# rsokolovskii/fl_scaling_sc_ldpc

Hardware: AMD Instinct MI355X
Metric: MC codeword trials/sec, (4,8) SC-LDPC L=50 N=1000 eps=0.48 full BP (higher is better)
Workload: dtype u32

## Files before the change

fl_scaling_sc_ldpc_amd/csrc/sampler_v2.hip:

```cpp
#include "common.h"
#include "kernel_util.h"
#include "philox.h"
#include <algorithm>
#include <cstdlib>

namespace {

using scldpc_dev::philox4x32_10;
using scldpc_dev::wave_inclusive_scan;

constexpr int kThreads = 1024;
constexpr int kWaves = kThreads / 64;
constexpr int kMaxDoped = 32;
constexpr int kWorkCap = 1024;

struct S2Args {
    int L, cns_pos, vns_pos, n, S, D, nb, shift, sbits, nw;
    int ntrials;
    int force_exact;
    int ndoped;
    int doped[kMaxDoped];
    uint32_t seed_lo, seed_hi;
    unsigned long long trial0;
    uint32_t thresh;
    int off_gpk, off_fix, off_stage, off_wsum;
    uint16_t *vn_adj16;
    uint16_t *cn_adj16;
    uint32_t *chan;
};

template <int KMAX, int ROWS, int CNMODE, bool PERSIST = false>
__global__ __launch_bounds__(kThreads, KMAX == 1 ? 8 : 4) __attribute__((amdgpu_num_sgpr(72))) void sample_philox_v2_kernel(const S2Args a)
{
    constexpr int DV = 4, DC_SHIFT = 3, E = 4 * KMAX;
    extern __shared__ uint32_t lds[];
    uint32_t *hist = lds;
    uint32_t *gpk = lds + a.off_gpk;
    uint16_t *fix = reinterpret_cast<uint16_t *>(lds + a.off_fix);
    uint16_t *stage = reinterpret_cast<uint16_t *>(lds + a.off_stage);
    uint32_t *wsum = lds + a.off_wsum;
    uint32_t *wl = wsum + 32;

    const int tid = threadIdx.x, lane = tid & 63, wave = tid >> 6;
    const int S = a.S, nb = a.nb;
    const int ncalls = S >> 2;
    const int kshift = a.shift - 2;
    const uint32_t lowmask = (1u << kshift) - 1u;
    bool own[KMAX];
#pragma unroll
    for (int k = 0; k < KMAX; k++) own[k] = tid + k * kThreads < ncalls;
    auto sock = [&](int e) { return (uint32_t)((tid + (e >> 2) * kThreads) * 4 + (e & 3)); };
    auto stage_entry = [&](int p, uint32_t sck) -> uint16_t {
        const int u = (int)(sck & 3u), t = (int)(sck >> 2);
        if ((unsigned)(p - u) >= (unsigned)a.L) return (uint16_t)0xFFFFu;
        return CNMODE == 1 ? (uint16_t)((p - u) * a.vns_pos + t) : (uint16_t)sck;
    };

    auto nib_sum = [](uint32_t x) {
        const uint32_t v = (x & 0x0F0Fu) + ((x >> 4) & 0x0F0Fu);
        return (v + (v >> 8)) & 0xFFu;
    };
    auto load_words = [&](uint32_t (&x)[ROWS]) {
        if constexpr (ROWS % 4 == 0) {
#pragma unroll
            for (int r = 0; r < ROWS / 4; r++) {
                const uint4 q = reinterpret_cast<const uint4 *>(hist)[tid * (ROWS / 4) + r];
                x[4 * r] = q.x; x[4 * r + 1] = q.y; x[4 * r + 2] = q.z; x[4 * r + 3] = q.w;
            }
        } else if constexpr (ROWS == 2) { const uint2 q = reinterpret_cast<const uint2 *>(hist)[tid]; x[0] = q.x; x[1] = q.y; }
        else x[0] = hist[tid];
    };
    auto store_words = [&](const uint32_t (&x)[ROWS]) {
        if constexpr (ROWS % 4 == 0) {
#pragma unroll
            for (int r = 0; r < ROWS / 4; r++)
                reinterpret_cast<uint4 *>(hist)[tid * (ROWS / 4) + r] = make_uint4(x[4 * r], x[4 * r + 1], x[4 * r + 2], x[4 * r + 3]);
        } else if constexpr (ROWS == 2) reinterpret_cast<uint2 *>(hist)[tid] = make_uint2(x[0], x[1]);
        else hist[tid] = x[0];
    };
    STAMP_DECL
    for (int b = tid; b < nb; b += kThreads) hist[b] = 0;
    if (tid == 0) { wsum[kWaves] = 0; wsum[kWaves + 1] = 0; }
    __syncthreads();
    auto sample_trial = [&](const int tr) {
    const unsigned long long trial = a.trial0 + (unsigned long long)tr;
    const uint32_t t_lo = (uint32_t)trial, t_hi = (uint32_t)(trial >> 32);
    uint32_t rowP[KMAX], rowQ[KMAX], rowR[KMAX];
#pragma unroll
    for (int k = 0; k < KMAX; k++) rowP[k] = rowQ[k] = rowR[k] = 0;
    uint32_t nxt[E];
#pragma unroll
    for (int k = 0; k < KMAX; k++) {
        uint32_t r[4] = {0, 0, 0, 0};
        if (own[k]) philox4x32_10((uint32_t)(tid + k * kThreads), 0u, t_lo, t_hi, a.seed_lo, a.seed_hi, r);
#pragma unroll
        for (int u = 0; u < 4; u++) nxt[4 * k + u] = r[u];
    }
    for (int p = 0; p < a.D; p++) {
        STAMP(0);
        uint32_t key[E], slot[E], crowded = 0;
#pragma unroll
        for (int e = 0; e < E; e++) {
            key[e] = nxt[e];
            const uint32_t b = key[e] >> kshift, sh = (b & 3u) * 4u;
            slot[e] = (atomicAdd(&hist[b >> 2], (own[e >> 2] ? 1u : 0u) << sh) >> sh) & 0xFu;
            crowded = max(crowded, slot[e]);
        }
        if (crowded >= 15u) wsum[kWaves + 1] = 1u;
        __syncthreads();
        STAMP(1);

        {
            uint32_t x[ROWS], v[ROWS], tot = 0;
            load_words(x);
#pragma unroll
            for (int r = 0; r < ROWS; r++) v[r] = 0;
            if constexpr (ROWS % 2 == 0) {
#pragma unroll
                for (int r = 0; r < ROWS; r += 2) {
                    const uint32_t y = x[r] | (x[r + 1] << 16);
                    const uint32_t sb = (y & 0x0F0F0F0Fu) + ((y >> 4) & 0x0F0F0F0Fu);
                    v[r] = (sb & 0xFFu) + ((sb >> 8) & 0xFFu);
                    v[r + 1] = ((sb >> 16) & 0xFFu) + (sb >> 24);
                    tot += v[r] + v[r + 1];
                }
            } else {
                static_assert(ROWS == 1 || ROWS % 2 == 0, "ROWS is 1, 2, 4 or 8");
                v[0] = nib_sum(x[0]);
                tot = v[0];
            }
            const uint32_t inc = wave_inclusive_scan(tot);
            if (lane == 63) wsum[wave] = inc;
            __syncthreads();
            const uint32_t wt = lane < kWaves ? wsum[lane] : 0u;
            const uint32_t winc = wave_inclusive_scan(wt);
            uint32_t pre = inc - tot + (uint32_t)__builtin_amdgcn_readlane((int)(winc - wt), wave);
#pragma unroll
            for (int r = 0; r < ROWS; r++) { x[r] |= pre << 16; pre += v[r]; }
            store_words(x);
        }
        __syncthreads();
        STAMP(2);

        if (wsum[kWaves + 1] == 0u) {
            uint32_t h[E], rk[E], g0a[E], cnta[E], smask = 0;
#pragma unroll
            for (int e = 0; e < E; e++) h[e] = hist[own[e >> 2] ? (key[e] >> kshift) >> 2 : 0u];
#pragma unroll
            for (int e = 0; e < E; e++) {
                const uint32_t k4 = ((key[e] >> kshift) & 3u) * 4u, x = h[e];
                const uint32_t below = x & ((1u << k4) - 1u);
                g0a[e] = (x >> 16) + (below & 0xFu) + ((below >> 4) & 0xFu) + ((below >> 8) & 0xFu);
                cnta[e] = (x >> k4) & 0xFu;
                rk[e] = g0a[e] + slot[e];
                if (own[e >> 2] && ((g0a[e] + cnta[e] - 1u) >> DC_SHIFT) != (g0a[e] >> DC_SHIFT)) smask |= 1u << e;
            }
            while (smask) {
                const uint32_t e = (uint32_t)__ffs((int)smask) - 1u;
                smask &= smask - 1u;
                uint32_t ky = key[0], sl = slot[0], g0 = g0a[0], cnt = cnta[0];
#pragma unroll
                for (int f = 1; f < E; f++)
                    if (e == (uint32_t)f) { ky = key[f]; sl = slot[f]; g0 = g0a[f]; cnt = cnta[f]; }
                const uint32_t pk = ((ky & lowmask) << a.sbits) | (uint32_t)((tid + (int)(e >> 2) * kThreads) * 4 + (int)(e & 3u));
                gpk[g0 + sl] = pk;
                const int w = atomicAdd(reinterpret_cast<int *>(&wsum[kWaves]), 1);
                if (w < kWorkCap) { wl[2 * w] = g0 | (cnt << 16) | (sl << 20); wl[2 * w + 1] = pk; }
            }
#pragma unroll
            for (int k = 0; k < KMAX; k++) {
                if (!own[k]) continue;
                uint2 v;
                v.x = (rk[4 * k] >> DC_SHIFT) | ((rk[4 * k + 1] >> DC_SHIFT) << 16);
                v.y = (rk[4 * k + 2] >> DC_SHIFT) | ((rk[4 * k + 3] >> DC_SHIFT) << 16);
                reinterpret_cast<uint2 *>(fix)[tid + k * kThreads] = v;
            }
            if constexpr (CNMODE != 0) {
#pragma unroll
                for (int k = 0; k < KMAX; k++) {
                    if (!own[k]) continue;
#pragma unroll
                    for (int u = 0; u < 4; u++) stage[rk[4 * k + u]] = stage_entry(p, sock(4 * k + u));
                }
            }
        }
        __syncthreads();
        STAMP(3);

        {
            uint32_t z[ROWS];
#pragma unroll
            for (int r = 0; r < ROWS; r++) z[r] = 0;
            store_words(z);
            int nwork = (int)wsum[kWaves];
            const bool exact = wsum[kWaves + 1] != 0u || nwork > kWorkCap || a.force_exact == p || a.force_exact == -2;
            if (exact) {
                nwork = 0;
#pragma unroll
                for (int e = 0; e < E; e++) if (own[e >> 2]) gpk[sock(e)] = key[e];
                __syncthreads();
                uint32_t xr[E];
#pragma unroll
                for (int e = 0; e < E; e++) xr[e] = 0;
                for (int s2 = 0; s2 < S; s2++) {
                    const uint32_t k2 = gpk[s2];
#pragma unroll
                    for (int e = 0; e < E; e++) xr[e] += (k2 < key[e]) || (k2 == key[e] && (uint32_t)s2 < sock(e));
                }
#pragma unroll
                for (int k = 0; k < KMAX; k++) {
                    if (!own[k]) continue;
                    uint2 v;
                    v.x = (xr[4 * k] >> DC_SHIFT) | ((xr[4 * k + 1] >> DC_SHIFT) << 16);
                    v.y = (xr[4 * k + 2] >> DC_SHIFT) | ((xr[4 * k + 3] >> DC_SHIFT) << 16);
                    reinterpret_cast<uint2 *>(fix)[tid + k * kThreads] = v;
                    if constexpr (CNMODE != 0) {
#pragma unroll
                        for (int u = 0; u < 4; u++) stage[xr[4 * k + u]] = stage_entry(p, sock(4 * k + u));
                    }
                }
            }
            for (int w = tid; w < nwork; w += kThreads) {
                const uint32_t ea = wl[2 * w], pk = wl[2 * w + 1];
                const uint32_t g0 = ea & 0xFFFFu, cnt = (ea >> 16) & 0xFu, sl = ea >> 20;
                uint32_t r = g0;
                for (uint32_t m = 0; m < cnt; m++)
                    if (m != sl) r += gpk[g0 + m] < pk;
                const uint32_t sck = pk & ((1u << a.sbits) - 1u);
                if constexpr (CNMODE != 0) stage[r] = stage_entry(p, sck);
                fix[sck] = (uint16_t)(r >> DC_SHIFT);
            }
        }
        if (p + 1 < a.D) {
            uint32_t k_lo = a.seed_lo, k_hi = a.seed_hi;
            asm volatile("" : "+s"(k_lo), "+s"(k_hi));
#pragma unroll
            for (int k = 0; k < KMAX; k++) {
                uint32_t r[4] = {0, 0, 0, 0};
                if (own[k]) philox4x32_10((uint32_t)(tid + k * kThreads), (uint32_t)(p + 1), t_lo, t_hi, k_lo, k_hi, r);
#pragma unroll
                for (int u = 0; u < 4; u++) nxt[4 * k + u] = r[u];
            }
        }
        __syncthreads();
        if (tid == 0) { wsum[kWaves] = 0; wsum[kWaves + 1] = 0; }
        STAMP(4);

        const int qpos = p - (DV - 1);
#pragma unroll
        for (int k = 0; k < KMAX; k++) {
            uint2 c = make_uint2(0u, 0u);
            if (own[k]) c = reinterpret_cast<const uint2 *>(fix)[tid + k * kThreads];
            if (qpos >= 0 && own[k]) {
                const size_t j = (size_t)tr * a.n + (size_t)qpos * a.vns_pos + (size_t)(tid + k * kThreads);
                uint2 v;
                v.x = rowP[k];
                v.y = (rowR[k] >> 16) | (c.y & 0xFFFF0000u);
                reinterpret_cast<uint2 *>(a.vn_adj16)[j] = v;
            }
            rowP[k] = rowQ[k];
            rowQ[k] = (rowR[k] & 0xFFFFu) | (c.x & 0xFFFF0000u);
            rowR[k] = (c.x & 0xFFFFu) | (c.y << 16);
        }
        if constexpr (CNMODE != 0) {
            uint2 *dst = reinterpret_cast<uint2 *>(a.cn_adj16) + ((size_t)tr * a.D + p) * (size_t)(S >> 2);
            const uint2 *src = reinterpret_cast<const uint2 *>(stage);
            for (int w = tid; w < (S >> 2); w += kThreads) dst[w] = src[w];
        }
        STAMP(5);
    }

    uint32_t *chan = a.chan + (size_t)tr * a.nw;
    for (int w = tid; w < a.nw; w += kThreads) {
        uint32_t word = 0;
#pragma unroll
        for (int c = 0; c < 8; c++) {
            uint32_t r[4];
            philox4x32_10((uint32_t)(w * 8 + c), 0x80000000u, t_lo, t_hi, a.seed_lo, a.seed_hi, r);
#pragma unroll
            for (int u = 0; u < 4; u++) word |= (uint32_t)((r[u] >> 1) < a.thresh) << (c * 4 + u);
        }
        const int j0 = w * 32;
        if (j0 + 32 > a.n) word &= (1u << (a.n - j0)) - 1u;
        for (int d = 0; d < a.ndoped; d++) {
            const int lo = max(a.doped[d] * a.vns_pos, j0) - j0, hi = min((a.doped[d] + 1) * a.vns_pos, j0 + 32) - j0;
            if (lo < hi) word &= ~(((hi - lo) == 32 ? 0xFFFFFFFFu : ((1u << (hi - lo)) - 1u)) << lo);
        }
        chan[w] = word;
    }
    STAMP(6);
    };
    if constexpr (PERSIST) {
        for (int tr = blockIdx.x; tr < a.ntrials; tr += gridDim.x) {
            sample_trial(tr);
            __syncthreads();
        }
    } else {
        sample_trial((int)blockIdx.x);
    }
    STAMP_FLUSH();
}


__device__ __forceinline__ uint32_t wl_entry_vn(const S2Args &a, int p, uint32_t sck)
{
    return (uint32_t)((p - (int)(sck & 3u)) * a.vns_pos + (int)(sck >> 2));
}

template <int LG, int CNMODE>
__global__ __launch_bounds__(kThreads, 8) __attribute__((amdgpu_num_sgpr(72))) void sample_philox_v3_kernel(const S2Args a)
{
    constexpr int DV = 4, DC_SHIFT = 3, E = 4;
    constexpr int NB = 1 << LG, ROWS = NB / kThreads;
    constexpr int KSHIFT = 32 - LG - 2;
    constexpr uint32_t LOWMASK = (1u << KSHIFT) - 1u;
    constexpr int SBITS = LG;
    static_assert(ROWS == 1 || ROWS == 2 || ROWS == 4, "one Philox call per thread: at most 4096 sockets per position");
    extern __shared__ uint32_t lds[];
    uint32_t *hist0 = lds;
    uint32_t *gpk = lds + a.off_gpk;
    uint16_t *fix = reinterpret_cast<uint16_t *>(lds + a.off_fix);
    uint16_t *stage = reinterpret_cast<uint16_t *>(lds + a.off_stage);
    uint32_t *wsum = lds + a.off_wsum;
    uint32_t *wl = wsum + 32;

    const int tid = threadIdx.x, lane = tid & 63, wave = tid >> 6;
    const int S = a.S;
    const bool own = tid < (S >> 2);
    const unsigned long long trial = a.trial0 + blockIdx.x;
    const uint32_t t_lo = (uint32_t)trial, t_hi = (uint32_t)(trial >> 32);
    const int tr = blockIdx.x;

    STAMP_DECL
    for (int b = tid; b < 2 * NB; b += kThreads) hist0[b] = 0;
    if (tid < 32) wsum[tid] = 0;
    __syncthreads();

    uint32_t rowP = 0, rowQ = 0, rowR = 0;
    uint32_t key[E] = {0, 0, 0, 0}, slot[E] = {0, 0, 0, 0};
    uint32_t ent0 = CNMODE == 1 ? (uint32_t)tid : (uint32_t)(4 * tid);
    uint32_t vV = (uint32_t)a.vns_pos;
    asm volatile("" : "+v"(vV));

    for (int p = 0; p <= a.D; p++) {
        uint32_t *hc = hist0 + (p & 1) * NB, *hp = hist0 + ((p & 1) ^ 1) * NB;
        const bool live = p < a.D;
        STAMP(0);
        if (p > 0) {
            int nwork = (int)wsum[16];
            const bool exact = wsum[18 + ((p - 1) & 1)] != 0u || nwork > kWorkCap || a.force_exact == p - 1 || a.force_exact == -2;
            if (exact) {
                uint32_t k2[4] = {0, 0, 0, 0};
                uint32_t f_lo = a.seed_lo, f_hi = a.seed_hi;
                asm volatile("" : "+s"(f_lo), "+s"(f_hi));
                if (own) philox4x32_10((uint32_t)tid, (uint32_t)(p - 1), t_lo, t_hi, f_lo, f_hi, k2);
                if (own) { gpk[4 * tid] = k2[0]; gpk[4 * tid + 1] = k2[1]; gpk[4 * tid + 2] = k2[2]; gpk[4 * tid + 3] = k2[3]; }
                __syncthreads();
                uint32_t xr[4] = {0, 0, 0, 0};
                for (int s2 = 0; s2 < S; s2++) {
                    const uint32_t kk = gpk[s2];
#pragma unroll
                    for (int u = 0; u < 4; u++) xr[u] += (kk < k2[u]) || (kk == k2[u] && s2 < 4 * tid + u);
                }
                if (own) {
                    uint2 v;
                    v.x = (xr[0] >> DC_SHIFT) | ((xr[1] >> DC_SHIFT) << 16);
                    v.y = (xr[2] >> DC_SHIFT) | ((xr[3] >> DC_SHIFT) << 16);
                    reinterpret_cast<uint2 *>(fix)[tid] = v;
                    if constexpr (CNMODE != 0) {
#pragma unroll
                        for (int u = 0; u < 4; u++) {
                            const int pu = p - 1 - u;
                            stage[xr[u]] = (unsigned)pu < (unsigned)a.L ? (uint16_t)(CNMODE == 1 ? pu * a.vns_pos + tid : 4 * tid + u) : (uint16_t)0xFFFFu;
                        }
                    }
                }
                nwork = 0;
            }
            for (int w = tid; w < nwork; w += kThreads) {
                const uint32_t ea = wl[2 * w], pk = wl[2 * w + 1];
                const uint32_t g0 = ea & 0xFFFFu, cnt = (ea >> 16) & 0xFu, sl = (ea >> 20) & 0xFu;
                uint32_t r = g0;
                for (uint32_t m = 0; m < cnt; m++)
                    if (m != sl) r += gpk[g0 + m] < pk;
                const uint32_t sck = pk & ((1u << SBITS) - 1u);
                if constexpr (CNMODE != 0) stage[r] = (uint16_t)(ea >> 24 ? 0xFFFFu : (CNMODE == 1 ? wl_entry_vn(a, p - 1, sck) : sck));
                fix[sck] = (uint16_t)(r >> DC_SHIFT);
            }
            {
                if constexpr (ROWS == 4) reinterpret_cast<uint4 *>(hp)[tid] = make_uint4(0u, 0u, 0u, 0u);
                else if constexpr (ROWS == 2) reinterpret_cast<uint2 *>(hp)[tid] = make_uint2(0u, 0u);
                else hp[tid] = 0u;
            }
        }
        STAMP(1);
        if (live) {
            {
                uint32_t k_lo = a.seed_lo, k_hi = a.seed_hi;
                asm volatile("" : "+s"(k_lo), "+s"(k_hi));
                uint32_t r[4] = {0, 0, 0, 0};
                if (own) philox4x32_10((uint32_t)tid, (uint32_t)p, t_lo, t_hi, k_lo, k_hi, r);
#pragma unroll
                for (int u = 0; u < 4; u++) key[u] = r[u];
            }
            uint32_t crowded = 0;
#pragma unroll
            for (int e = 0; e < E; e++) {
                const uint32_t boff = (key[e] >> KSHIFT) & ~3u, sh = (key[e] >> (KSHIFT - 2)) & 12u;
                const uint32_t old = atomicAdd(reinterpret_cast<uint32_t *>(reinterpret_cast<char *>(hc) + boff), (own ? 16u : 0u) << sh);
                slot[e] = (old >> (sh + 4u)) & 0xFu;
                crowded |= slot[e] + 1u;
            }
            if (crowded & 16u) wsum[18 + (p & 1)] = 1u;
        }
        STAMP(2);
        __syncthreads();
        STAMP(3);
        if (tid == 0) { wsum[16] = 0; wsum[18 + ((p & 1) ^ 1)] = 0; }
        if (live) {
            uint32_t x[ROWS], tot = 0, over = 0;
            if constexpr (ROWS == 4) { const uint4 q = reinterpret_cast<const uint4 *>(hc)[tid]; x[0] = q.x; x[1] = q.y; x[2] = q.z; x[3] = q.w; }
            else if constexpr (ROWS == 2) { const uint2 q = reinterpret_cast<const uint2 *>(hc)[tid]; x[0] = q.x; x[1] = q.y; }
            else x[0] = hc[tid];
            uint32_t v[ROWS];
#pragma unroll
            for (int r = 0; r < ROWS; r++) {
                const uint32_t y = x[r] * 0x1111u;
                const uint32_t sb = (x[r] & 0x0F0F0u) + ((x[r] >> 4) & 0x0F0F0u);
                v[r] = ((sb + (sb >> 8)) >> 4) & 0xFFu;
                over |= v[r];
                x[r] = y & 0xFFFF0u;
                tot += v[r];
            }
            if (over & ~15u) wsum[18 + (p & 1)] = 1u;
            const uint32_t inc = wave_inclusive_scan(tot);
            uint32_t pre = inc - tot;
#pragma unroll
            for (int r = 0; r < ROWS; r++) { x[r] |= pre << 20; pre += v[r]; }
            if constexpr (ROWS == 4) reinterpret_cast<uint4 *>(hc)[tid] = make_uint4(x[0], x[1], x[2], x[3]);
            else if constexpr (ROWS == 2) reinterpret_cast<uint2 *>(hc)[tid] = make_uint2(x[0], x[1]);
            else hc[tid] = x[0];
            if (lane == 63) wsum[wave] = inc;
        }
        if (p > 0) {
            const int pp = p - 1, qpos = pp - (DV - 1);
            uint2 c = make_uint2(0u, 0u);
            if (own) c = reinterpret_cast<const uint2 *>(fix)[tid];
            if (qpos >= 0 && own) {
                const size_t j = (size_t)tr * a.n + (size_t)qpos * a.vns_pos + (size_t)tid;
                uint2 vv;
                vv.x = rowP;
                vv.y = (rowR >> 16) | (c.y & 0xFFFF0000u);
                reinterpret_cast<uint2 *>(a.vn_adj16)[j] = vv;
            }
            rowP = rowQ;
            rowQ = (rowR & 0xFFFFu) | (c.x & 0xFFFF0000u);
            rowR = (c.x & 0xFFFFu) | (c.y << 16);
            if constexpr (CNMODE != 0) {
                uint2 *dst = reinterpret_cast<uint2 *>(a.cn_adj16) + ((size_t)tr * a.D + pp) * (size_t)(S >> 2);
                const uint2 *src = reinterpret_cast<const uint2 *>(stage);
                if (own) dst[tid] = src[tid];
            }
        }
        STAMP(4);
        __syncthreads();
        STAMP(5);
        if (live && wsum[18 + (p & 1)] == 0u) {
            const uint32_t wt = lane < kWaves ? wsum[lane] : 0u;
            uint32_t wi = wt;
            wi += (uint32_t)__builtin_amdgcn_update_dpp(0, (int)wi, 0x111, 0xF, 0xF, false);
            wi += (uint32_t)__builtin_amdgcn_update_dpp(0, (int)wi, 0x112, 0xF, 0xF, false);
            wi += (uint32_t)__builtin_amdgcn_update_dpp(0, (int)wi, 0x114, 0xF, 0xF, false);
            wi += (uint32_t)__builtin_amdgcn_update_dpp(0, (int)wi, 0x118, 0xF, 0xF, false);
            const uint32_t wex = wi - wt;
            uint32_t h[E], wb[E], rk[E], g0a[E], cnta[E];
#pragma unroll
            for (int e = 0; e < E; e++) h[e] = *reinterpret_cast<const uint32_t *>(reinterpret_cast<const char *>(hc) + ((key[e] >> KSHIFT) & ~3u));
#pragma unroll
            for (int e = 0; e < E; e++) wb[e] = (uint32_t)__builtin_amdgcn_ds_bpermute((int)((key[e] >> 26) & 0x3Cu), (int)wex);
            bool st[E];
            bool anyst = false;
#pragma unroll
            for (int e = 0; e < E; e++) {
                const uint32_t t1 = h[e] >> ((key[e] >> (KSHIFT - 2)) & 12u);
                const uint32_t excl = t1 & 15u, incl = (t1 >> 4) & 15u;
                g0a[e] = (h[e] >> 20) + wb[e] + excl;
                cnta[e] = incl - excl;
                rk[e] = g0a[e] + slot[e];
                st[e] = own && ((g0a[e] ^ (g0a[e] + cnta[e] - 1u)) >> DC_SHIFT) != 0u;
                anyst = anyst || st[e];
            }
            if (own) {
                uint2 vv;
                vv.x = (rk[0] >> DC_SHIFT) | ((rk[1] >> DC_SHIFT) << 16);
                vv.y = (rk[2] >> DC_SHIFT) | ((rk[3] >> DC_SHIFT) << 16);
                reinterpret_cast<uint2 *>(fix)[tid] = vv;
            }
            const bool edge = p < DV - 1 || p >= a.L;
            if constexpr (CNMODE != 0) {
                if (own) {
                    uint32_t ent[E];
                    ent[0] = ent0;
#pragma unroll
                    for (int u = 1; u < 4; u++) ent[u] = CNMODE == 1 ? ent[u - 1] - vV : ent[u - 1] + 1u;
                    if (!edge) {
#pragma unroll
                        for (int u = 0; u < 4; u++) stage[rk[u]] = (uint16_t)ent[u];
                    } else {
#pragma unroll
                        for (int u = 0; u < 4; u++) stage[rk[u]] = (unsigned)(p - u) < (unsigned)a.L ? (uint16_t)ent[u] : (uint16_t)0xFFFFu;
                    }
                }
            }
            if (__builtin_amdgcn_ballot_w64(anyst)) {
                unsigned long long vote[E];
                int total = 0;
#pragma unroll
                for (int e = 0; e < E; e++) { vote[e] = __builtin_amdgcn_ballot_w64(st[e]); total += __builtin_popcountll(vote[e]); }
                int base = 0;
                if (lane == 0) base = atomicAdd(reinterpret_cast<int *>(&wsum[16]), total);
                base = __builtin_amdgcn_readfirstlane(base);
#pragma unroll
                for (int e = 0; e < E; e++) {
                    if (st[e]) {
                        const int w = base + (int)__builtin_amdgcn_mbcnt_hi((uint32_t)(vote[e] >> 32), __builtin_amdgcn_mbcnt_lo((uint32_t)vote[e], 0u));
                        const uint32_t pk = ((key[e] & LOWMASK) << SBITS) | (uint32_t)(4 * tid + e);
                        gpk[g0a[e] + slot[e]] = pk;
                        const uint32_t none = CNMODE != 0 && edge && !((unsigned)(p - e) < (unsigned)a.L) ? 1u : 0u;
                        if (w < kWorkCap) { wl[2 * w] = g0a[e] | (cnta[e] << 16) | (slot[e] << 20) | (none << 24); wl[2 * w + 1] = pk; }
                    }
                    base += __builtin_popcountll(vote[e]);
                }
            }
        }
        if constexpr (CNMODE == 1) ent0 += vV;
        STAMP(6);
        __syncthreads();
        STAMP(7);
    }

    uint32_t *chan = a.chan + (size_t)tr * a.nw;
    for (int w = tid; w < a.nw; w += kThreads) {
        uint32_t word = 0;
        uint32_t c_lo = a.seed_lo, c_hi = a.seed_hi;
        asm volatile("" : "+s"(c_lo), "+s"(c_hi));
#pragma unroll
        for (int c = 0; c < 8; c++) {
            uint32_t r[4];
            philox4x32_10((uint32_t)(w * 8 + c), 0x80000000u, t_lo, t_hi, c_lo, c_hi, r);
#pragma unroll
            for (int u = 0; u < 4; u++) word |= (uint32_t)((r[u] >> 1) < a.thresh) << (c * 4 + u);
        }
        const int j0 = w * 32;
        if (j0 + 32 > a.n) word &= (1u << (a.n - j0)) - 1u;
        for (int d = 0; d < a.ndoped; d++) {
            const int lo = max(a.doped[d] * a.vns_pos, j0) - j0, hi = min((a.doped[d] + 1) * a.vns_pos, j0 + 32) - j0;
            if (lo < hi) word &= ~(((hi - lo) == 32 ? 0xFFFFFFFFu : ((1u << (hi - lo)) - 1u)) << lo);
        }
        chan[w] = word;
    }
    STAMP(8);
    STAMP_FLUSH();
}

int launch_v2(const char *who, int cnmode, const scldpc_code_params *p, uint64_t seed, uint64_t trial0, int32_t ntrials,
              double eps, int32_t ndoped, const int32_t *doped_positions, uint16_t *d_vn_adj16, uint16_t *d_table,
              uint32_t *d_chan_bits, void *stream)
{
    if (ntrials < 0 || (ntrials > 0 && (!d_vn_adj16 || !d_chan_bits)))
        return scldpc::set_error(SCLDPC_ERR_BAD_ARG, "%s: null buffer or negative ntrials", who);
    if (ndoped < 0 || ndoped > kMaxDoped || (ndoped > 0 && !doped_positions))
        return scldpc::set_error(SCLDPC_ERR_BAD_ARG, "%s: 0 <= ndoped <= %d", who, kMaxDoped);
    if (!(eps >= 0.0 && eps <= 1.0))
        return scldpc::set_error(SCLDPC_ERR_BAD_ARG, "%s: eps=%g outside [0,1]", who, eps);
    if (ntrials == 0) return SCLDPC_OK;
    if (!d_table) cnmode = 0;

    S2Args a{};
    a.L = p->L; a.cns_pos = p->cns_pos; a.vns_pos = p->vns_pos;
    a.n = scldpc::n_of(p); a.S = p->cns_pos * p->dc; a.D = p->L + p->dv - 1; a.nw = scldpc::nw_of(p);
    int lg = 10;
    while ((1 << lg) < a.S) lg++;
    a.nb = 1 << lg; a.shift = 32 - lg; a.sbits = lg;
    a.ndoped = ndoped;
    for (int d = 0; d < ndoped; d++) {
        if (doped_positions[d] < 0 || doped_positions[d] >= p->L)
            return scldpc::set_error(SCLDPC_ERR_BAD_ARG, "doped position %d outside [0,%d)", doped_positions[d], p->L);
        a.doped[d] = doped_positions[d];
    }
    a.seed_lo = (uint32_t)seed; a.seed_hi = (uint32_t)(seed >> 32);
    a.trial0 = trial0;
    {
        const double x = eps * 2147483647.0;
        double c = (double)(uint64_t)x;
        if (c < x) c += 1.0;
        a.thresh = (uint32_t)c;
    }
    const char *gen_env = getenv("SCLDPC_SAMPLER_GEN");
    const bool v3 = a.nb <= 4 * kThreads && gen_env && atoi(gen_env) == 3;
    int off = ((v3 ? 2 : 1) * a.nb + 3) & ~3;
    a.off_gpk = off;   off += (a.S + 3) & ~3;
    a.off_fix = off;   off += (a.S / 2 + 3) & ~3;
    a.off_stage = off; off += cnmode ? (a.S / 2 + 3) & ~3 : 0;
    a.off_wsum = off;  off += 32 + 2 * kWorkCap;
    size_t lds_bytes = 4u * (size_t)off;
    lds_bytes = std::min(lds_bytes + scldpc::debug_lds_pad("SAMPLER"), std::max(lds_bytes, (size_t)scldpc::kMaxLdsBytes));
    if (lds_bytes > (size_t)scldpc::kMaxLdsBytes)
        return scldpc::set_error(SCLDPC_ERR_TOO_LARGE, "%s: %zu bytes of LDS per trial", who, lds_bytes);
    a.vn_adj16 = d_vn_adj16; a.cn_adj16 = d_table; a.chan = d_chan_bits;
    a.ntrials = ntrials;
    a.force_exact = -1;
    if (const char *v = getenv("SCLDPC_DEBUG_SAMPLER_EXACT_POS")) a.force_exact = atoi(v);

    using Kern = void (*)(const S2Args);
    static const Kern table[4][3] = {
        {sample_philox_v2_kernel<1, 1, 0>, sample_philox_v2_kernel<1, 1, 1>, sample_philox_v2_kernel<1, 1, 2>},
        {sample_philox_v2_kernel<1, 2, 0>, sample_philox_v2_kernel<1, 2, 1>, sample_philox_v2_kernel<1, 2, 2>},
        {sample_philox_v2_kernel<1, 4, 0>, sample_philox_v2_kernel<1, 4, 1>, sample_philox_v2_kernel<1, 4, 2>},
        {sample_philox_v2_kernel<2, 8, 0>, sample_philox_v2_kernel<2, 8, 1>, sample_philox_v2_kernel<2, 8, 2>},
    };
    const int rows = a.nb / kThreads;
    static const Kern table3[3][3] = {
        {sample_philox_v3_kernel<10, 0>, sample_philox_v3_kernel<10, 1>, sample_philox_v3_kernel<10, 2>},
        {sample_philox_v3_kernel<11, 0>, sample_philox_v3_kernel<11, 1>, sample_philox_v3_kernel<11, 2>},
        {sample_philox_v3_kernel<12, 0>, sample_philox_v3_kernel<12, 1>, sample_philox_v3_kernel<12, 2>},
    };
    const int grid = v3 ? ntrials : scldpc::debug_grid("SAMPLER", ntrials);
    Kern kern = v3 ? table3[lg - 10][cnmode] : table[rows == 1 ? 0 : rows == 2 ? 1 : rows == 4 ? 2 : 3][cnmode];
    if (grid < ntrials && rows == 4 && cnmode == 1) kern = sample_philox_v2_kernel<1, 4, 1, true>;
    else if (grid < ntrials) return scldpc::set_error(SCLDPC_ERR_BAD_ARG, "SCLDPC_DEBUG_GRID_SAMPLER: only the <1,4,1> kernel has a persistent form");
    if (int rc_ = scldpc::allow_max_lds(reinterpret_cast<const void *>(kern))) return rc_;
    hipLaunchKernelGGL(kern, dim3(grid), dim3(kThreads), lds_bytes, static_cast<hipStream_t>(stream), a);
    SCLDPC_HIP_CHECK(hipGetLastError());
    return SCLDPC_OK;
}

bool v2_shape(const scldpc_code_params *p)
{
    if (scldpc::check_params(p)) return false;
    const int S = p->cns_pos * p->dc;
    return p->dv == 4 && p->dc == 8 && (S & 3) == 0 && S <= 8192 && p->vns_pos * p->dv == S;
}

}

extern "C" int scldpc_sample_philox_cn16_supported(const scldpc_code_params *p)
{
    return v2_shape(p) && scldpc::n_of(p) < 65535;
}

extern "C" int scldpc_sample_philox_sock16_supported(const scldpc_code_params *p)
{
    return v2_shape(p);
}

extern "C" int scldpc_sample_philox_device_cn16(const scldpc_code_params *p, uint64_t seed, uint64_t trial0,
                                                int32_t ntrials, double eps, int32_t ndoped,
                                                const int32_t *doped_positions, uint16_t *d_vn_adj16,
                                                uint16_t *d_cn_adj16, uint32_t *d_chan_bits, void *stream)
{
    const char *who = "scldpc_sample_philox_device_cn16";
    if (int rc = scldpc::check_params(p)) return rc;
    if (!scldpc_sample_philox_cn16_supported(p))
        return scldpc::set_error(SCLDPC_ERR_TOO_LARGE, "%s: takes dv = 4, dc = 8, at most 8192 sockets per position and "
                                 "fewer than 65535 VNs (got dv=%d dc=%d cns_pos=%d n=%d)", who, p->dv, p->dc, p->cns_pos,
                                 scldpc::n_of(p));
    return launch_v2(who, 1, p, seed, trial0, ntrials, eps, ndoped, doped_positions, d_vn_adj16, d_cn_adj16, d_chan_bits,
                     stream);
}

extern "C" int scldpc_sample_philox_device_sock16(const scldpc_code_params *p, uint64_t seed, uint64_t trial0,
                                                  int32_t ntrials, double eps, int32_t ndoped,
                                                  const int32_t *doped_positions, uint16_t *d_vn_adj16,
                                                  uint16_t *d_cn_sock16, uint32_t *d_chan_bits, void *stream)
{
    const char *who = "scldpc_sample_philox_device_sock16";
    if (int rc = scldpc::check_params(p)) return rc;
    if (!scldpc_sample_philox_sock16_supported(p))
        return scldpc::set_error(SCLDPC_ERR_TOO_LARGE, "%s: takes dv = 4, dc = 8 and at most 8192 sockets per position "
                                 "(got dv=%d dc=%d cns_pos=%d)", who, p->dv, p->dc, p->cns_pos);
    return launch_v2(who, 2, p, seed, trial0, ntrials, eps, ndoped, doped_positions, d_vn_adj16, d_cn_sock16, d_chan_bits,
                     stream);
}
```

Measured before the change: 1.138 million.

## Specialize sampler bucket math at compile time and use wave-aggregated worklist appends

Derives the bucket shift and width from the ROWS template parameter instead of runtime arguments, so key-to-word and nibble extraction become constant shifts. For KMAX==1 it replaces the nibble-sum prefix with a multiply-by-0x111110 inclusive nibble scan, and detects overflow by checking that the scanned total equals S instead of tracking a crowded flag. It appends straddling entries to the worklist with one ballot/mbcnt-based atomic per wave rather than one atomic per lane. The tie-resolution loop now compares against the whole bucket range, including the entry itself. This assumes the launched ROWS always matches the runtime nb and relies on the overflow check to catch nibble saturation.

```diff
diff --git a/fl_scaling_sc_ldpc_amd/csrc/sampler_v2.hip b/fl_scaling_sc_ldpc_amd/csrc/sampler_v2.hip
--- a/fl_scaling_sc_ldpc_amd/csrc/sampler_v2.hip
+++ b/fl_scaling_sc_ldpc_amd/csrc/sampler_v2.hip
@@ -15,7 +15,7 @@
 constexpr int kWorkCap = 1024;
 
 struct S2Args {
-    int L, cns_pos, vns_pos, n, S, D, nb, shift, sbits, nw;
+    int L, cns_pos, vns_pos, n, S, D, nb, nw;
     int ntrials;
     int force_exact;
     int ndoped;
@@ -33,6 +33,10 @@
 __global__ __launch_bounds__(kThreads, KMAX == 1 ? 8 : 4) __attribute__((amdgpu_num_sgpr(72))) void sample_philox_v2_kernel(const S2Args a)
 {
     constexpr int DV = 4, DC_SHIFT = 3, E = 4 * KMAX;
+    constexpr int LG = ROWS == 1 ? 10 : ROWS == 2 ? 11 : ROWS == 4 ? 12 : 13;
+    constexpr int KSHIFT = 32 - LG - 2;
+    constexpr bool INCL = KMAX == 1;
+    static_assert(ROWS * kThreads == (1 << LG) && (INCL ? ROWS <= 4 : ROWS == 8), "ROWS is 1, 2, 4 (KMAX 1) or 8 (KMAX 2)");
     extern __shared__ uint32_t lds[];
     uint32_t *hist = lds;
     uint32_t *gpk = lds + a.off_gpk;
@@ -44,8 +48,6 @@
     const int tid = threadIdx.x, lane = tid & 63, wave = tid >> 6;
     const int S = a.S, nb = a.nb;
     const int ncalls = S >> 2;
-    const int kshift = a.shift - 2;
-    const uint32_t lowmask = (1u << kshift) - 1u;
     bool own[KMAX];
 #pragma unroll
     for (int k = 0; k < KMAX; k++) own[k] = tid + k * kThreads < ncalls;
@@ -99,18 +101,48 @@
     for (int p = 0; p < a.D; p++) {
         STAMP(0);
         uint32_t key[E], slot[E], crowded = 0;
+        auto word_of = [](uint32_t k) { return (k >> KSHIFT) & ~3u; };
+        auto nib_of = [](uint32_t k) { return (k >> (KSHIFT - 2)) & 12u; };
 #pragma unroll
         for (int e = 0; e < E; e++) {
             key[e] = nxt[e];
-            const uint32_t b = key[e] >> kshift, sh = (b & 3u) * 4u;
-            slot[e] = (atomicAdd(&hist[b >> 2], (own[e >> 2] ? 1u : 0u) << sh) >> sh) & 0xFu;
-            crowded = max(crowded, slot[e]);
-        }
-        if (crowded >= 15u) wsum[kWaves + 1] = 1u;
+            const uint32_t sh = nib_of(key[e]);
+            uint32_t *w = reinterpret_cast<uint32_t *>(reinterpret_cast<char *>(hist) + word_of(key[e]));
+            slot[e] = (atomicAdd(w, (own[e >> 2] ? 1u : 0u) << sh) >> sh) & 0xFu;
+            if constexpr (!INCL) crowded = max(crowded, slot[e]);
+        }
+        if (!INCL && crowded >= 15u) wsum[kWaves + 1] = 1u;
         __syncthreads();
         STAMP(1);
 
-        {
+        bool ranked;
+        if constexpr (INCL) {
+            uint32_t x[ROWS], t20[ROWS], tot20 = 0;
+            load_words(x);
+#pragma unroll
+            for (int r = 0; r < ROWS; r++) {
+                x[r] *= 0x111110u;
+                t20[r] = x[r] & 0xF00000u;
+                tot20 += t20[r];
+            }
+            const uint32_t tot = tot20 >> 20, inc = wave_inclusive_scan(tot);
+            if (lane == 63) wsum[wave] = inc;
+            __syncthreads();
+            uint32_t winc = lane < kWaves ? wsum[lane] : 0u;
+            const uint32_t wt = winc;
+            winc += (uint32_t)__builtin_amdgcn_update_dpp(0, (int)winc, 0x111, 0xF, 0xF, false);
+            winc += (uint32_t)__builtin_amdgcn_update_dpp(0, (int)winc, 0x112, 0xF, 0xF, false);
+            winc += (uint32_t)__builtin_amdgcn_update_dpp(0, (int)winc, 0x114, 0xF, 0xF, false);
+            winc += (uint32_t)__builtin_amdgcn_update_dpp(0, (int)winc, 0x118, 0xF, 0xF, false);
+            ranked = __builtin_amdgcn_readlane((int)winc, kWaves - 1) == S;
+            uint32_t pre20 = (inc - tot + (uint32_t)__builtin_amdgcn_readlane((int)(winc - wt), wave)) << 20;
+#pragma unroll
+            for (int r = 0; r < ROWS; r++) {
+                x[r] = (x[r] & 0xFFFF0u) | pre20;
+                pre20 += t20[r];
+            }
+            store_words(x);
+        } else {
             uint32_t x[ROWS], v[ROWS], tot = 0;
             load_words(x);
 #pragma unroll
@@ -140,32 +172,76 @@
             store_words(x);
         }
         __syncthreads();
+        if constexpr (!INCL) ranked = wsum[kWaves + 1] == 0u;
         STAMP(2);
 
-        if (wsum[kWaves + 1] == 0u) {
-            uint32_t h[E], rk[E], g0a[E], cnta[E], smask = 0;
-#pragma unroll
-            for (int e = 0; e < E; e++) h[e] = hist[own[e >> 2] ? (key[e] >> kshift) >> 2 : 0u];
-#pragma unroll
-            for (int e = 0; e < E; e++) {
-                const uint32_t k4 = ((key[e] >> kshift) & 3u) * 4u, x = h[e];
-                const uint32_t below = x & ((1u << k4) - 1u);
-                g0a[e] = (x >> 16) + (below & 0xFu) + ((below >> 4) & 0xFu) + ((below >> 8) & 0xFu);
-                cnta[e] = (x >> k4) & 0xFu;
-                rk[e] = g0a[e] + slot[e];
-                if (own[e >> 2] && ((g0a[e] + cnta[e] - 1u) >> DC_SHIFT) != (g0a[e] >> DC_SHIFT)) smask |= 1u << e;
-            }
-            while (smask) {
-                const uint32_t e = (uint32_t)__ffs((int)smask) - 1u;
-                smask &= smask - 1u;
-                uint32_t ky = key[0], sl = slot[0], g0 = g0a[0], cnt = cnta[0];
-#pragma unroll
-                for (int f = 1; f < E; f++)
-                    if (e == (uint32_t)f) { ky = key[f]; sl = slot[f]; g0 = g0a[f]; cnt = cnta[f]; }
-                const uint32_t pk = ((ky & lowmask) << a.sbits) | (uint32_t)((tid + (int)(e >> 2) * kThreads) * 4 + (int)(e & 3u));
-                gpk[g0 + sl] = pk;
-                const int w = atomicAdd(reinterpret_cast<int *>(&wsum[kWaves]), 1);
-                if (w < kWorkCap) { wl[2 * w] = g0 | (cnt << 16) | (sl << 20); wl[2 * w + 1] = pk; }
+        if (ranked) {
+            uint32_t rk[E], g0a[E], g1a[E];
+            bool st[E];
+            if constexpr (INCL) {
+                uint32_t h[E];
+#pragma unroll
+                for (int e = 0; e < E; e++) h[e] = *reinterpret_cast<const uint32_t *>(reinterpret_cast<const char *>(hist) + word_of(key[e]));
+#pragma unroll
+                for (int e = 0; e < E; e++) {
+                    const uint32_t t = h[e] >> nib_of(key[e]), pre = h[e] >> 20;
+                    g0a[e] = pre + (t & 0xFu);
+                    g1a[e] = pre + ((t >> 4) & 0xFu);
+                    rk[e] = g0a[e] + slot[e];
+                    st[e] = own[e >> 2] && ((g0a[e] ^ (g1a[e] - 1u)) >> DC_SHIFT) != 0u;
+                }
+            } else {
+                uint32_t h[E];
+#pragma unroll
+                for (int e = 0; e < E; e++) h[e] = hist[own[e >> 2] ? (key[e] >> KSHIFT) >> 2 : 0u];
+#pragma unroll
+                for (int e = 0; e < E; e++) {
+                    const uint32_t k4 = ((key[e] >> KSHIFT) & 3u) * 4u, x = h[e];
+                    const uint32_t below = x & ((1u << k4) - 1u);
+                    g0a[e] = (x >> 16) + (below & 0xFu) + ((below >> 4) & 0xFu) + ((below >> 8) & 0xFu);
+                    g1a[e] = g0a[e] + ((x >> k4) & 0xFu);
+                    rk[e] = g0a[e] + slot[e];
+                    st[e] = own[e >> 2] && ((g1a[e] - 1u) >> DC_SHIFT) != (g0a[e] >> DC_SHIFT);
+                }
+            }
+            if constexpr (INCL) {
+                unsigned long long vote[E], anyv = 0;
+                int total = 0;
+#pragma unroll
+                for (int e = 0; e < E; e++) { vote[e] = __builtin_amdgcn_ballot_w64(st[e]); anyv |= vote[e]; total += __builtin_popcountll(vote[e]); }
+                if (anyv) {
+                    int base = 0;
+                    if (lane == 0) base = atomicAdd(reinterpret_cast<int *>(&wsum[kWaves]), total);
+                    base = __builtin_amdgcn_readfirstlane(base);
+                    const bool fits = base + total <= kWorkCap;
+#pragma unroll
+                    for (int e = 0; e < E; e++) {
+                        if (st[e]) {
+                            const uint32_t w = __builtin_amdgcn_mbcnt_hi((uint32_t)(vote[e] >> 32),
+                                                                         __builtin_amdgcn_mbcnt_lo((uint32_t)vote[e], (uint32_t)base));
+                            const uint32_t pk = (key[e] << LG) | sock(e);
+                            gpk[rk[e]] = pk;
+                            if (fits) { wl[2 * w] = g0a[e] | (g1a[e] << 16); wl[2 * w + 1] = pk; }
+                        }
+                        base += __builtin_popcountll(vote[e]);
+                    }
+                }
+            } else {
+                uint32_t smask = 0;
+#pragma unroll
+                for (int e = 0; e < E; e++) smask |= (st[e] ? 1u : 0u) << e;
+                while (smask) {
+                    const uint32_t e = (uint32_t)__ffs((int)smask) - 1u;
+                    smask &= smask - 1u;
+                    uint32_t ky = key[0], r0 = rk[0], g0 = g0a[0], g1 = g1a[0];
+#pragma unroll
+                    for (int f = 1; f < E; f++)
+                        if (e == (uint32_t)f) { ky = key[f]; r0 = rk[f]; g0 = g0a[f]; g1 = g1a[f]; }
+                    const uint32_t pk = (ky << LG) | (uint32_t)((tid + (int)(e >> 2) * kThreads) * 4 + (int)(e & 3u));
+                    gpk[r0] = pk;
+                    const int w = atomicAdd(reinterpret_cast<int *>(&wsum[kWaves]), 1);
+                    if (w < kWorkCap) { wl[2 * w] = g0 | (g1 << 16); wl[2 * w + 1] = pk; }
+                }
             }
 #pragma unroll
             for (int k = 0; k < KMAX; k++) {
@@ -193,8 +269,9 @@
             for (int r = 0; r < ROWS; r++) z[r] = 0;
             store_words(z);
             int nwork = (int)wsum[kWaves];
-            const bool exact = wsum[kWaves + 1] != 0u || nwork > kWorkCap || a.force_exact == p || a.force_exact == -2;
+            const bool exact = !ranked || nwork > kWorkCap || a.force_exact == p || a.force_exact == -2;
             if (exact) {
+                asm volatile("; ledger: cold");
                 nwork = 0;
 #pragma unroll
                 for (int e = 0; e < E; e++) if (own[e >> 2]) gpk[sock(e)] = key[e];
@@ -222,11 +299,10 @@
             }
             for (int w = tid; w < nwork; w += kThreads) {
                 const uint32_t ea = wl[2 * w], pk = wl[2 * w + 1];
-                const uint32_t g0 = ea & 0xFFFFu, cnt = (ea >> 16) & 0xFu, sl = ea >> 20;
-                uint32_t r = g0;
-                for (uint32_t m = 0; m < cnt; m++)
-                    if (m != sl) r += gpk[g0 + m] < pk;
-                const uint32_t sck = pk & ((1u << a.sbits) - 1u);
+                uint32_t r = ea & 0xFFFFu;
+#pragma unroll 1
+                for (uint32_t m = ea & 0xFFFFu; m < (ea >> 16); m++) r += gpk[m] < pk;
+                const uint32_t sck = pk & ((1u << LG) - 1u);
                 if constexpr (CNMODE != 0) stage[r] = stage_entry(p, sck);
                 fix[sck] = (uint16_t)(r >> DC_SHIFT);
             }
@@ -581,7 +657,7 @@
     a.n = scldpc::n_of(p); a.S = p->cns_pos * p->dc; a.D = p->L + p->dv - 1; a.nw = scldpc::nw_of(p);
     int lg = 10;
     while ((1 << lg) < a.S) lg++;
-    a.nb = 1 << lg; a.shift = 32 - lg; a.sbits = lg;
+    a.nb = 1 << lg;
     a.ndoped = ndoped;
     for (int d = 0; d < ndoped; d++) {
         if (doped_positions[d] < 0 || doped_positions[d] >= p->L)
```

After: 1.215 million (median of 6 runs). 1.07x the previous value.
